# IDEA-CCNL/Fengshenbang-LM

Hardware: NVIDIA H100
Metric: tokens_per_sec (higher is better)
Workload: dtype bf16

## Files before the change

### fengshen-lm_b200/csrc/attention_bwd.cu

```cuda
#include "host_common.h"
#include "ptx.cuh"

namespace fsb {

int make_attn_tmap(CUtensorMap* tm, const void* base, int64_t row_stride, int64_t width, int64_t seq, int64_t batch,
                   int box_rows);

constexpr int AB_THREADS = 384;
constexpr int AB_BM = 128;
constexpr int AB_BN = 64;
constexpr int AB_NDIAG = AB_BM + AB_BN - 1;
constexpr int AB_DSTRIDE = 192;

struct AttBwdParams {
  const float* lse;
  const float* delta;
  const uint8_t* kv_mask;
  const float* rel_bias;
  float* dbias_part;
  __nv_bfloat16 *dq, *dk, *dv;
  int64_t dq_row_stride, dk_row_stride, dv_row_stride, dq_head_stride, dk_head_stride, dv_head_stride;
  int q_head_stride, k_head_stride, v_head_stride, do_head_stride;
  int seq_q, seq_kv, nheads, batch, causal;
  float scale, scale_log2;
};

template <int D>
__global__ void __launch_bounds__(256) attn_delta_kernel(const __nv_bfloat16* __restrict__ o,
                                                         const __nv_bfloat16* __restrict__ dout, float* __restrict__ delta,
                                                         int64_t o_row_stride, int64_t o_head_stride,
                                                         int64_t do_row_stride, int64_t do_head_stride, int batch, int seq,
                                                         int nheads) {
  constexpr int G = D / 8;
  const int64_t gid = (blockIdx.x * int64_t(blockDim.x) + threadIdx.x) / G;
  const int gl = threadIdx.x % G;
  const int64_t total = int64_t(batch) * seq * nheads;
  float s = 0.f;
  int64_t bs = 0; int h = 0;
  if (gid < total) {
    h = int(gid % nheads);
    bs = gid / nheads;
    float a[8], b[8];
    unpack8(*reinterpret_cast<const uint4*>(o + bs * o_row_stride + h * o_head_stride + gl * 8), a);
    unpack8(*reinterpret_cast<const uint4*>(dout + bs * do_row_stride + h * do_head_stride + gl * 8), b);
#pragma unroll
    for (int j = 0; j < 8; ++j) s += a[j] * b[j];
  }
#pragma unroll
  for (int off = G / 2; off > 0; off >>= 1) s += __shfl_xor_sync(0xffffffffu, s, off);
  if (gid < total && gl == 0) {
    const int64_t b = bs / seq, sq = bs % seq;
    delta[(b * nheads + h) * seq + sq] = s;
  }
}

template <int D, bool kDS>
struct AttBwdSmem {
  static constexpr int BIG_BYTES = AB_BM * D * 2;
  static constexpr int SML_BYTES = AB_BN * D * 2;
  static constexpr int STAGES = 3;
  static constexpr int OFF_BIG0 = 0;
  static constexpr int OFF_BIG1 = OFF_BIG0 + BIG_BYTES;
  static constexpr int OFF_SML0 = OFF_BIG1 + BIG_BYTES;
  static constexpr int OFF_SML1 = OFF_SML0 + STAGES * SML_BYTES;
  static constexpr int OFF_DS = OFF_SML1 + STAGES * SML_BYTES;
  static constexpr int OFF_BAR = OFF_DS + (kDS ? (AB_BM * (AB_BN + 1) * 4 + 15) / 16 * 16 : 0);
  static constexpr int NBAR = 1 + 2 * STAGES;
  static constexpr int TOTAL = OFF_BAR + NBAR * 8 + 1024;
  static_assert(TOTAL <= 232448, "exceeds the 227 KB of shared memory a block can opt into on sm_90");
};

template <int D>
__device__ __forceinline__ void wgmma_rs_acc(float (&o)[D / 2], const uint32_t (&a)[4], uint64_t db) {
  if constexpr (D == 128) wgmma_rs_n128<1>(o, a, db, 1u);
  else wgmma_rs_n64<1>(o, a, db, 1u);
}
__device__ __forceinline__ uint32_t kslice(int kk, int rows) { return (kk / 4) * (rows * 128) + (kk % 4) * 32; }
__device__ __forceinline__ void to_frag(const float (&x)[32], int kk, uint32_t (&a)[4]) {
#pragma unroll
  for (int r = 0; r < 4; ++r) {
    const int i = 2 * kk + (r >> 1), h = r & 1;
    a[r] = pack_bf16x2(x[4 * i + 2 * h], x[4 * i + 2 * h + 1]);
  }
}

template <int D, bool kBias>
__global__ void __launch_bounds__(AB_THREADS, 1)
attn_bwd_dq_kernel(const __grid_constant__ CUtensorMap tmQ, const __grid_constant__ CUtensorMap tmdO,
                   const __grid_constant__ CUtensorMap tmK, const __grid_constant__ CUtensorMap tmV,
                   const AttBwdParams p) {
  using S = AttBwdSmem<D, kBias>;
  constexpr int STAGES = S::STAGES;
  extern __shared__ uint8_t smem_raw[];
  uint8_t* smem = reinterpret_cast<uint8_t*>((reinterpret_cast<uintptr_t>(smem_raw) + 1023) & ~uintptr_t(1023));
  uint64_t* bars = reinterpret_cast<uint64_t*>(smem + S::OFF_BAR);
  uint64_t* big_full = bars;
  uint64_t* sml_full = big_full + 1;
  uint64_t* sml_empty = sml_full + STAGES;

  const int warp = threadIdx.x >> 5, lane = threadIdx.x & 31;
  const int tile = gridDim.x - 1 - blockIdx.x;
  const int head = blockIdx.y, b = blockIdx.z;
  const int q0 = tile * AB_BM;
  const int n_all = (p.seq_kv + AB_BN - 1) / AB_BN;
  const int n_steps = p.causal ? min(n_all, (min(q0 + AB_BM, p.seq_q) + AB_BN - 1) / AB_BN) : n_all;

  if (threadIdx.x == 0) {
    tma_prefetch_desc(&tmQ); tma_prefetch_desc(&tmdO); tma_prefetch_desc(&tmK); tma_prefetch_desc(&tmV);
    mbar_init(big_full, 1);
    for (int i = 0; i < STAGES; ++i) { mbar_init(&sml_full[i], 1); mbar_init(&sml_empty[i], 8); }
    fence_barrier_init();
  }
  __syncthreads();

  if (warp < 4) {
    reg_dec<24>();
    if (threadIdx.x == 0) {
      const int qc = head * p.q_head_stride, dc = head * p.do_head_stride;
      const int kc = head * p.k_head_stride, vc = head * p.v_head_stride;
      mbar_expect_tx(big_full, 2 * S::BIG_BYTES);
#pragma unroll
      for (int h = 0; h < D / 64; ++h) {
        tma_load_3d(smem + S::OFF_BIG0 + h * (AB_BM * 128), &tmQ, big_full, qc + h * 64, q0, b);
        tma_load_3d(smem + S::OFF_BIG1 + h * (AB_BM * 128), &tmdO, big_full, dc + h * 64, q0, b);
      }
      int st = 0; uint32_t ph = 0;
      for (int j = 0; j < n_steps; ++j) {
        mbar_wait(&sml_empty[st], ph ^ 1);
        mbar_expect_tx(&sml_full[st], 2 * S::SML_BYTES);
#pragma unroll
        for (int h = 0; h < D / 64; ++h) {
          tma_load_3d(smem + S::OFF_SML0 + st * S::SML_BYTES + h * (AB_BN * 128), &tmK, &sml_full[st], kc + h * 64, j * AB_BN, b);
          tma_load_3d(smem + S::OFF_SML1 + st * S::SML_BYTES + h * (AB_BN * 128), &tmV, &sml_full[st], vc + h * 64, j * AB_BN, b);
        }
        if (++st == STAGES) { st = 0; ph ^= 1; }
      }
    }
    return;
  }

  reg_inc<240>();
  const int wg = (threadIdx.x >> 7) - 1;
  const int r_lo = wg * 64 + (warp & 3) * 16 + (lane >> 2);
  const int cq = 2 * (lane & 3);
  const uint64_t dsc_q = make_smem_desc_sw128(smem_u32(smem + S::OFF_BIG0) + wg * (64 * 128), 0, 1024);
  const uint64_t dsc_do = make_smem_desc_sw128(smem_u32(smem + S::OFF_BIG1) + wg * (64 * 128), 0, 1024);
  const uint64_t dsc_k = make_smem_desc_sw128(smem_u32(smem + S::OFF_SML0), 0, 1024);
  const uint64_t dsc_v = make_smem_desc_sw128(smem_u32(smem + S::OFF_SML1), 0, 1024);
  const uint64_t dsc_kmn = make_smem_desc_sw128(smem_u32(smem + S::OFF_SML0), AB_BN * 128, 1024);
  const uint8_t* mrow = p.kv_mask ? p.kv_mask + int64_t(b) * p.seq_kv : nullptr;
  const int n_rel = p.seq_q + p.seq_kv - 1;
  int q_row[2], kmax[2];
  float lse[2], delta[2];
  const float* brow[2];
#pragma unroll
  for (int h = 0; h < 2; ++h) {
    q_row[h] = q0 + r_lo + 8 * h;
    const bool ok = q_row[h] < p.seq_q;
    const int64_t si = (int64_t(b) * p.nheads + head) * p.seq_q + q_row[h];
    lse[h] = ok ? p.lse[si] : INFINITY;
    delta[h] = ok ? p.delta[si] : 0.f;
    kmax[h] = p.causal ? min(q_row[h], p.seq_kv - 1) : p.seq_kv - 1;
    brow[h] = kBias ? p.rel_bias + int64_t(head) * n_rel + (p.seq_q - 1 - min(q_row[h], p.seq_q - 1)) : nullptr;
  }
  float* dpart = kBias && p.dbias_part ? p.dbias_part + ((int64_t(b) * p.nheads + head) * gridDim.x + tile) * n_all * AB_DSTRIDE
                                       : nullptr;
  float dq[D / 2];
#pragma unroll
  for (int i = 0; i < D / 2; ++i) dq[i] = 0.f;

  mbar_wait(big_full, 0);
  for (int j = 0; j < n_steps; ++j) {
    const int st = j % STAGES;
    const uint32_t ph = (j / STAGES) & 1;
    const uint64_t sto = uint64_t(st) * (S::SML_BYTES >> 4);
    float s[32], dp[32];
    mbar_wait(&sml_full[st], ph);
    wgmma_fence();
#pragma unroll
    for (int kk = 0; kk < D / 16; ++kk)
      wgmma_ss_n64<0, 0>(s, dsc_q + (kslice(kk, AB_BM) >> 4), dsc_k + sto + (kslice(kk, AB_BN) >> 4), kk != 0 ? 1u : 0u);
#pragma unroll
    for (int kk = 0; kk < D / 16; ++kk)
      wgmma_ss_n64<0, 0>(dp, dsc_do + (kslice(kk, AB_BM) >> 4), dsc_v + sto + (kslice(kk, AB_BN) >> 4), kk != 0 ? 1u : 0u);
    wgmma_commit();
    wgmma_wait<0>();
    wgmma_fence_acc(s);
    wgmma_fence_acc(dp);
    const int c0 = j * AB_BN;
    const bool need_mask = (p.causal && c0 + AB_BN - 1 > q0 + wg * 64) || (c0 + AB_BN > p.seq_kv) || mrow;
#pragma unroll
    for (int i = 0; i < 8; ++i) {
#pragma unroll
      for (int e = 0; e < 4; ++e) {
        const int h = e >> 1, col = c0 + 8 * i + cq + (e & 1);
        float x = s[4 * i + e] * p.scale_log2 - lse[h];
        if constexpr (kBias) x = fmaf(__ldg(brow[h] + min(col, p.seq_kv - 1)), 1.4426950408889634f, x);
        float pe = ex2_approx(x);
        if (need_mask) {
          bool keep = col <= kmax[h];
          if (mrow != nullptr && keep) keep = mrow[col] != 0;
          pe = keep ? pe : 0.f;
        }
        s[4 * i + e] = pe * (dp[4 * i + e] - delta[h]);
      }
    }
    if constexpr (kBias) {
      if (dpart != nullptr) {
        float* tds = reinterpret_cast<float*>(smem + S::OFF_DS);
#pragma unroll
        for (int i = 0; i < 8; ++i)
#pragma unroll
          for (int e = 0; e < 4; ++e) tds[(r_lo + 8 * (e >> 1)) * (AB_BN + 1) + 8 * i + cq + (e & 1)] = s[4 * i + e];
        bar_sync(1, 256);
        const int t = threadIdx.x - 128;
        if (t < AB_NDIAG) {
          const int o = t - (AB_BM - 1);
          float acc = 0.f;
          for (int r = max(0, -o); r < min(AB_BM, AB_BN - o); ++r) acc += tds[r * (AB_BN + 2) + o];
          dpart[int64_t(j) * AB_DSTRIDE + t] = acc;
        }
        bar_sync(1, 256);
      }
    }
    uint32_t a[AB_BN / 16][4];
#pragma unroll
    for (int kk = 0; kk < AB_BN / 16; ++kk) to_frag(s, kk, a[kk]);
    wgmma_fence();
#pragma unroll
    for (int kk = 0; kk < AB_BN / 16; ++kk) wgmma_rs_acc<D>(dq, a[kk], dsc_kmn + sto + ((kk * 2048) >> 4));
    wgmma_commit();
    wgmma_wait<0>();
    wgmma_fence_acc(dq);
    __syncwarp();
    if (lane == 0) mbar_arrive(&sml_empty[st]);
  }
#pragma unroll
  for (int h = 0; h < 2; ++h) {
    if (q_row[h] >= p.seq_q) continue;
    __nv_bfloat16* dqp = p.dq + (int64_t(b) * p.seq_q + q_row[h]) * p.dq_row_stride + int64_t(head) * p.dq_head_stride + cq;
#pragma unroll
    for (int i = 0; i < D / 8; ++i)
      *reinterpret_cast<uint32_t*>(dqp + 8 * i) = pack_bf16x2(dq[4 * i + 2 * h] * p.scale, dq[4 * i + 2 * h + 1] * p.scale);
  }
}

template <int D, bool kBias>
__global__ void __launch_bounds__(AB_THREADS, 1)
attn_bwd_dkv_kernel(const __grid_constant__ CUtensorMap tmK, const __grid_constant__ CUtensorMap tmV,
                    const __grid_constant__ CUtensorMap tmQ, const __grid_constant__ CUtensorMap tmdO,
                    const AttBwdParams p) {
  using S = AttBwdSmem<D, false>;
  constexpr int STAGES = S::STAGES;
  extern __shared__ uint8_t smem_raw[];
  uint8_t* smem = reinterpret_cast<uint8_t*>((reinterpret_cast<uintptr_t>(smem_raw) + 1023) & ~uintptr_t(1023));
  uint64_t* bars = reinterpret_cast<uint64_t*>(smem + S::OFF_BAR);
  uint64_t* big_full = bars;
  uint64_t* sml_full = big_full + 1;
  uint64_t* sml_empty = sml_full + STAGES;

  const int warp = threadIdx.x >> 5, lane = threadIdx.x & 31;
  const int tile = blockIdx.x;
  const int head = blockIdx.y, b = blockIdx.z;
  const int kv0 = tile * AB_BM;
  const int n_q = (p.seq_q + AB_BN - 1) / AB_BN;
  const int i_start = p.causal ? min(n_q, kv0 / AB_BN) : 0;
  const int n_steps = n_q - i_start;

  if (threadIdx.x == 0) {
    tma_prefetch_desc(&tmQ); tma_prefetch_desc(&tmdO); tma_prefetch_desc(&tmK); tma_prefetch_desc(&tmV);
    mbar_init(big_full, 1);
    for (int i = 0; i < STAGES; ++i) { mbar_init(&sml_full[i], 1); mbar_init(&sml_empty[i], 8); }
    fence_barrier_init();
  }
  __syncthreads();

  if (warp < 4) {
    reg_dec<24>();
    if (threadIdx.x == 0) {
      const int qc = head * p.q_head_stride, dc = head * p.do_head_stride;
      const int kc = head * p.k_head_stride, vc = head * p.v_head_stride;
      mbar_expect_tx(big_full, 2 * S::BIG_BYTES);
#pragma unroll
      for (int h = 0; h < D / 64; ++h) {
        tma_load_3d(smem + S::OFF_BIG0 + h * (AB_BM * 128), &tmK, big_full, kc + h * 64, kv0, b);
        tma_load_3d(smem + S::OFF_BIG1 + h * (AB_BM * 128), &tmV, big_full, vc + h * 64, kv0, b);
      }
      int st = 0; uint32_t ph = 0;
      for (int i = 0; i < n_steps; ++i) {
        mbar_wait(&sml_empty[st], ph ^ 1);
        mbar_expect_tx(&sml_full[st], 2 * S::SML_BYTES);
#pragma unroll
        for (int h = 0; h < D / 64; ++h) {
          tma_load_3d(smem + S::OFF_SML0 + st * S::SML_BYTES + h * (AB_BN * 128), &tmQ, &sml_full[st], qc + h * 64,
                      (i_start + i) * AB_BN, b);
          tma_load_3d(smem + S::OFF_SML1 + st * S::SML_BYTES + h * (AB_BN * 128), &tmdO, &sml_full[st], dc + h * 64,
                      (i_start + i) * AB_BN, b);
        }
        if (++st == STAGES) { st = 0; ph ^= 1; }
      }
    }
    return;
  }

  reg_inc<240>();
  const int wg = (threadIdx.x >> 7) - 1;
  const int r_lo = wg * 64 + (warp & 3) * 16 + (lane >> 2);
  const int cq = 2 * (lane & 3);
  const uint64_t dsc_k = make_smem_desc_sw128(smem_u32(smem + S::OFF_BIG0) + wg * (64 * 128), 0, 1024);
  const uint64_t dsc_v = make_smem_desc_sw128(smem_u32(smem + S::OFF_BIG1) + wg * (64 * 128), 0, 1024);
  const uint64_t dsc_q = make_smem_desc_sw128(smem_u32(smem + S::OFF_SML0), 0, 1024);
  const uint64_t dsc_do = make_smem_desc_sw128(smem_u32(smem + S::OFF_SML1), 0, 1024);
  const uint64_t dsc_qmn = make_smem_desc_sw128(smem_u32(smem + S::OFF_SML0), AB_BN * 128, 1024);
  const uint64_t dsc_domn = make_smem_desc_sw128(smem_u32(smem + S::OFF_SML1), AB_BN * 128, 1024);
  const int64_t stat_base = (int64_t(b) * p.nheads + head) * p.seq_q;
  const int n_rel = p.seq_q + p.seq_kv - 1;
  int kv_row[2];
  bool row_ok[2];
  const float* bkey[2];
#pragma unroll
  for (int h = 0; h < 2; ++h) {
    kv_row[h] = kv0 + r_lo + 8 * h;
    row_ok[h] = kv_row[h] < p.seq_kv && (p.kv_mask == nullptr || p.kv_mask[int64_t(b) * p.seq_kv + kv_row[h]] != 0);
    bkey[h] = kBias ? p.rel_bias + int64_t(head) * n_rel + (min(kv_row[h], p.seq_kv - 1) + p.seq_q - 1) : nullptr;
  }
  float dv[D / 2], dk[D / 2];
#pragma unroll
  for (int i = 0; i < D / 2; ++i) { dv[i] = 0.f; dk[i] = 0.f; }

  mbar_wait(big_full, 0);
  for (int i = 0; i < n_steps; ++i) {
    const int st = i % STAGES;
    const uint32_t ph = (i / STAGES) & 1;
    const uint64_t sto = uint64_t(st) * (S::SML_BYTES >> 4);
    const int qt0 = (i_start + i) * AB_BN;
    float s[32], dp[32];
    mbar_wait(&sml_full[st], ph);
    wgmma_fence();
#pragma unroll
    for (int kk = 0; kk < D / 16; ++kk)
      wgmma_ss_n64<0, 0>(s, dsc_k + (kslice(kk, AB_BM) >> 4), dsc_q + sto + (kslice(kk, AB_BN) >> 4), kk != 0 ? 1u : 0u);
#pragma unroll
    for (int kk = 0; kk < D / 16; ++kk)
      wgmma_ss_n64<0, 0>(dp, dsc_v + (kslice(kk, AB_BM) >> 4), dsc_do + sto + (kslice(kk, AB_BN) >> 4), kk != 0 ? 1u : 0u);
    wgmma_commit();
    wgmma_wait<0>();
    wgmma_fence_acc(s);
    wgmma_fence_acc(dp);
    const bool need_causal = p.causal && (qt0 < kv0 + AB_BM - 1);
#pragma unroll
    for (int ii = 0; ii < 8; ++ii) {
#pragma unroll
      for (int c = 0; c < 2; ++c) {
        const int qi = qt0 + 8 * ii + cq + c;
        const bool q_ok = qi < p.seq_q;
        const float lse_c = q_ok ? __ldg(p.lse + stat_base + qi) : INFINITY;
        const float del_c = q_ok ? __ldg(p.delta + stat_base + qi) : 0.f;
#pragma unroll
        for (int h = 0; h < 2; ++h) {
          const int e = 2 * h + c;
          float arg = s[4 * ii + e] * p.scale_log2 - lse_c;
          if constexpr (kBias) arg = fmaf(__ldg(bkey[h] - min(qi, p.seq_q - 1)), 1.4426950408889634f, arg);
          float x = ex2_approx(arg);
          const bool keep = row_ok[h] && !(need_causal && qi < kv_row[h]);
          x = keep ? x : 0.f;
          s[4 * ii + e] = x;
          dp[4 * ii + e] = x * (dp[4 * ii + e] - del_c);
        }
      }
    }
    uint32_t pa[AB_BN / 16][4], da[AB_BN / 16][4];
#pragma unroll
    for (int kk = 0; kk < AB_BN / 16; ++kk) { to_frag(s, kk, pa[kk]); to_frag(dp, kk, da[kk]); }
    wgmma_fence();
#pragma unroll
    for (int kk = 0; kk < AB_BN / 16; ++kk) wgmma_rs_acc<D>(dv, pa[kk], dsc_domn + sto + ((kk * 2048) >> 4));
#pragma unroll
    for (int kk = 0; kk < AB_BN / 16; ++kk) wgmma_rs_acc<D>(dk, da[kk], dsc_qmn + sto + ((kk * 2048) >> 4));
    wgmma_commit();
    wgmma_wait<0>();
    wgmma_fence_acc(dv);
    wgmma_fence_acc(dk);
    __syncwarp();
    if (lane == 0) mbar_arrive(&sml_empty[st]);
  }
#pragma unroll
  for (int h = 0; h < 2; ++h) {
    if (kv_row[h] >= p.seq_kv) continue;
    __nv_bfloat16* dvp = p.dv + (int64_t(b) * p.seq_kv + kv_row[h]) * p.dv_row_stride + int64_t(head) * p.dv_head_stride + cq;
    __nv_bfloat16* dkp = p.dk + (int64_t(b) * p.seq_kv + kv_row[h]) * p.dk_row_stride + int64_t(head) * p.dk_head_stride + cq;
#pragma unroll
    for (int i = 0; i < D / 8; ++i) {
      *reinterpret_cast<uint32_t*>(dvp + 8 * i) = pack_bf16x2(dv[4 * i + 2 * h], dv[4 * i + 2 * h + 1]);
      *reinterpret_cast<uint32_t*>(dkp + 8 * i) = pack_bf16x2(dk[4 * i + 2 * h] * p.scale, dk[4 * i + 2 * h + 1] * p.scale);
    }
  }
}

__global__ void __launch_bounds__(128) attn_dbias_reduce_kernel(const float* __restrict__ part, float* __restrict__ part2,
                                                                int batch, int nheads, int seq_q, int seq_kv, int causal,
                                                                int n_qtiles, int bsplit) {
  const int n_rel = seq_q + seq_kv - 1;
  const int i = blockIdx.x * blockDim.x + threadIdx.x;
  const int h = blockIdx.y, sp = blockIdx.z;
  if (i >= n_rel) return;
  const int d = i - (seq_q - 1);
  const int n_all = (seq_kv + AB_BN - 1) / AB_BN;
  const int b0 = int(int64_t(batch) * sp / bsplit), b1 = int(int64_t(batch) * (sp + 1) / bsplit);
  float acc = 0.f;
  for (int b = b0; b < b1; ++b) {
    for (int tile = 0; tile < n_qtiles; ++tile) {
      const int q0 = tile * AB_BM;
      const int n_steps = causal ? min(n_all, (min(q0 + AB_BM, seq_q) + AB_BN - 1) / AB_BN) : n_all;
      const float* base = part + ((int64_t(b) * nheads + h) * n_qtiles + tile) * n_all * AB_DSTRIDE;
      const int hi = d + q0 + (AB_BM - 1), lo = d + q0 - (AB_BN - 1);
      if (hi < 0) continue;
      const int j_lo = lo <= 0 ? 0 : (lo + AB_BN - 1) / AB_BN, j_hi = min(n_steps - 1, hi / AB_BN);
      for (int j = j_lo; j <= j_hi; ++j) acc += base[int64_t(j) * AB_DSTRIDE + (hi - j * AB_BN)];
    }
  }
  part2[(int64_t(sp) * nheads + h) * n_rel + i] = acc;
}
__global__ void __launch_bounds__(128) attn_dbias_final_kernel(const float* __restrict__ part2, float* __restrict__ dbias,
                                                               int nheads, int n_rel, int bsplit) {
  const int i = blockIdx.x * blockDim.x + threadIdx.x;
  const int h = blockIdx.y;
  if (i >= n_rel) return;
  float acc = dbias[int64_t(h) * n_rel + i];
  for (int sp = 0; sp < bsplit; ++sp) acc += part2[(int64_t(sp) * nheads + h) * n_rel + i];
  dbias[int64_t(h) * n_rel + i] = acc;
}
static inline int dbias_bsplit(int batch) { return batch < 16 ? batch : 16; }
static inline size_t dbias_part_floats(int64_t batch, int64_t seq_q, int64_t seq_kv, int nheads) {
  const int64_t n_qt = (seq_q + AB_BM - 1) / AB_BM, n_all = (seq_kv + AB_BN - 1) / AB_BN;
  return size_t(batch) * nheads * n_qt * n_all * AB_DSTRIDE;
}

template <int D, bool kBias>
static int launch_attn_bwd(const void* q, const void* k, const void* v, const void* o, const void* dout,
                           int64_t q_rs, int64_t k_rs, int64_t v_rs, int64_t o_rs, int64_t do_rs, int64_t o_hs,
                           float* delta, AttBwdParams& p, float* drel_bias, float* part2, cudaStream_t st) {
  using SQ = AttBwdSmem<D, kBias>;
  using SK = AttBwdSmem<D, false>;
  static bool configured = false;
  if (!configured) {
    cudaError_t e1 = cudaFuncSetAttribute(attn_bwd_dq_kernel<D, kBias>, cudaFuncAttributeMaxDynamicSharedMemorySize, SQ::TOTAL);
    cudaError_t e2 = cudaFuncSetAttribute(attn_bwd_dkv_kernel<D, kBias>, cudaFuncAttributeMaxDynamicSharedMemorySize, SK::TOTAL);
    if (e1 != cudaSuccess || e2 != cudaSuccess) {
      set_error("sdpa_bwd: cudaFuncSetAttribute(%d / %d) failed", SQ::TOTAL, SK::TOTAL);
      return FSB_ERR_CUDA;
    }
    configured = true;
  }
  {
    const int64_t groups = int64_t(p.batch) * p.seq_q * p.nheads;
    const int64_t threads = groups * (D / 8);
    attn_delta_kernel<D><<<unsigned((threads + 255) / 256), 256, 0, st>>>(
        (const __nv_bfloat16*)o, (const __nv_bfloat16*)dout, delta, o_rs, o_hs, do_rs, p.do_head_stride, p.batch, p.seq_q,
        p.nheads);
    FSB_CUDA_LAUNCH_CHECK();
  }
  CUtensorMap tq128, tdo128, tk64, tv64, tk128, tv128, tq64, tdo64;
  int rc;
  const int64_t wq = int64_t(p.nheads - 1) * p.q_head_stride + D, wk = int64_t(p.nheads - 1) * p.k_head_stride + D;
  const int64_t wv = int64_t(p.nheads - 1) * p.v_head_stride + D, wdo = int64_t(p.nheads - 1) * p.do_head_stride + D;
  if ((rc = make_attn_tmap(&tq128, q, q_rs, wq, p.seq_q, p.batch, AB_BM))) return rc;
  if ((rc = make_attn_tmap(&tdo128, dout, do_rs, wdo, p.seq_q, p.batch, AB_BM))) return rc;
  if ((rc = make_attn_tmap(&tk64, k, k_rs, wk, p.seq_kv, p.batch, AB_BN))) return rc;
  if ((rc = make_attn_tmap(&tv64, v, v_rs, wv, p.seq_kv, p.batch, AB_BN))) return rc;
  if ((rc = make_attn_tmap(&tk128, k, k_rs, wk, p.seq_kv, p.batch, AB_BM))) return rc;
  if ((rc = make_attn_tmap(&tv128, v, v_rs, wv, p.seq_kv, p.batch, AB_BM))) return rc;
  if ((rc = make_attn_tmap(&tq64, q, q_rs, wq, p.seq_q, p.batch, AB_BN))) return rc;
  if ((rc = make_attn_tmap(&tdo64, dout, do_rs, wdo, p.seq_q, p.batch, AB_BN))) return rc;
  {
    dim3 grid((p.seq_q + AB_BM - 1) / AB_BM, p.nheads, p.batch);
    attn_bwd_dq_kernel<D, kBias><<<grid, AB_THREADS, SQ::TOTAL, st>>>(tq128, tdo128, tk64, tv64, p);
    FSB_CUDA_LAUNCH_CHECK();
    if (kBias && drel_bias != nullptr) {
      const int n_rel = p.seq_q + p.seq_kv - 1, bs = dbias_bsplit(p.batch);
      attn_dbias_reduce_kernel<<<dim3((n_rel + 127) / 128, p.nheads, bs), 128, 0, st>>>(
          p.dbias_part, part2, p.batch, p.nheads, p.seq_q, p.seq_kv, p.causal, int(grid.x), bs);
      FSB_CUDA_LAUNCH_CHECK();
      attn_dbias_final_kernel<<<dim3((n_rel + 127) / 128, p.nheads), 128, 0, st>>>(part2, drel_bias, p.nheads, n_rel, bs);
      FSB_CUDA_LAUNCH_CHECK();
    }
  }
  {
    dim3 grid((p.seq_kv + AB_BM - 1) / AB_BM, p.nheads, p.batch);
    attn_bwd_dkv_kernel<D, kBias><<<grid, AB_THREADS, SK::TOTAL, st>>>(tk128, tv128, tq64, tdo64, p);
    FSB_CUDA_LAUNCH_CHECK();
  }
  return FSB_OK;
}

}

using namespace fsb;

extern "C" int fsb_sdpa_bwd(const void* q, const void* k, const void* v, const void* o, const void* dout,
                            const float* lse, float* delta, void* dq, void* dk, void* dv, int64_t batch, int64_t seq_q,
                            int64_t seq_kv, int nheads, int head_dim, int64_t q_row_stride, int64_t k_row_stride,
                            int64_t v_row_stride, int64_t o_row_stride, int64_t do_row_stride, int64_t dq_row_stride,
                            int64_t dk_row_stride, int64_t dv_row_stride, int64_t q_head_stride, int64_t k_head_stride,
                            int64_t v_head_stride, int64_t o_head_stride, int64_t do_head_stride,
                            int64_t dq_head_stride, int64_t dk_head_stride, int64_t dv_head_stride, float scale,
                            int causal, const uint8_t* kv_mask, const float* rel_bias, float* drel_bias, void* workspace,
                            size_t workspace_bytes, fsb_stream_t st) {
  FSB_REQUIRE(q && k && v && o && dout && lse && delta && dq && dk && dv, "sdpa_bwd: null pointer");
  FSB_REQUIRE(head_dim == 64 || head_dim == 128, "sdpa_bwd: head_dim %d unsupported (64 or 128)", head_dim);
  FSB_REQUIRE(batch > 0 && seq_q > 0 && seq_kv > 0 && nheads > 0 && batch < 65536 && nheads < 65536, "sdpa_bwd: bad dims");
  FSB_REQUIRE(!causal || seq_q == seq_kv, "sdpa_bwd: causal needs seq_q == seq_kv");
  FSB_REQUIRE(aligned16(q) && aligned16(k) && aligned16(v) && aligned16(o) && aligned16(dout) && aligned16(dq) &&
                  aligned16(dk) && aligned16(dv),
              "sdpa_bwd: 16-byte alignment required");
  FSB_REQUIRE((q_row_stride | k_row_stride | v_row_stride | o_row_stride | do_row_stride | dq_row_stride |
               dk_row_stride | dv_row_stride | q_head_stride | k_head_stride | v_head_stride | o_head_stride |
               do_head_stride | dq_head_stride | dk_head_stride | dv_head_stride) % 8 == 0,
              "sdpa_bwd: strides must be multiples of 8 elements");
  FSB_REQUIRE(drel_bias == nullptr || rel_bias != nullptr, "sdpa_bwd: drel_bias without rel_bias");
  AttBwdParams p;
  p.lse = lse; p.delta = delta; p.kv_mask = kv_mask;
  p.rel_bias = rel_bias; p.dbias_part = nullptr;
  float* part2 = nullptr;
  if (drel_bias != nullptr) {
    const size_t need = fsb_sdpa_bwd_workspace_bytes(batch, seq_q, seq_kv, nheads);
    FSB_REQUIRE(workspace != nullptr && workspace_bytes >= need && aligned16(workspace),
                "sdpa_bwd: the bias gradient needs a %zu-byte workspace (fsb_sdpa_bwd_workspace_bytes); got %zu", need,
                workspace_bytes);
    p.dbias_part = static_cast<float*>(workspace);
    part2 = p.dbias_part + dbias_part_floats(batch, seq_q, seq_kv, nheads);
  }
  p.dq = (__nv_bfloat16*)dq; p.dk = (__nv_bfloat16*)dk; p.dv = (__nv_bfloat16*)dv;
  p.dq_row_stride = dq_row_stride; p.dk_row_stride = dk_row_stride; p.dv_row_stride = dv_row_stride;
  p.dq_head_stride = dq_head_stride; p.dk_head_stride = dk_head_stride; p.dv_head_stride = dv_head_stride;
  p.q_head_stride = int(q_head_stride); p.k_head_stride = int(k_head_stride); p.v_head_stride = int(v_head_stride);
  p.do_head_stride = int(do_head_stride);
  p.seq_q = int(seq_q); p.seq_kv = int(seq_kv); p.nheads = nheads; p.batch = int(batch); p.causal = causal;
  p.scale = scale; p.scale_log2 = scale * 1.4426950408889634f;
#define FSB_BWD(DD, BB)                                                                                                  \
  launch_attn_bwd<DD, BB>(q, k, v, o, dout, q_row_stride, k_row_stride, v_row_stride, o_row_stride, do_row_stride,       \
                          o_head_stride, delta, p, drel_bias, part2, (cudaStream_t)st)
  if (rel_bias != nullptr) return head_dim == 128 ? FSB_BWD(128, true) : FSB_BWD(64, true);
  return head_dim == 128 ? FSB_BWD(128, false) : FSB_BWD(64, false);
#undef FSB_BWD
}

extern "C" size_t fsb_sdpa_bwd_workspace_bytes(int64_t batch, int64_t seq_q, int64_t seq_kv, int nheads) {
  if (batch <= 0 || seq_q <= 0 || seq_kv <= 0 || nheads <= 0) return 0;
  return (fsb::dbias_part_floats(batch, seq_q, seq_kv, nheads) +
          size_t(fsb::dbias_bsplit(int(batch))) * nheads * size_t(seq_q + seq_kv - 1)) * sizeof(float);
}
```

### fengshen-lm_b200/csrc/ptx.cuh

```cuda
#pragma once
#include <cuda.h>
#include <cuda_bf16.h>
#include <cuda_runtime.h>
#include <stdint.h>

namespace fsb {

__device__ __forceinline__ uint32_t smem_u32(const void* p) {
  return static_cast<uint32_t>(__cvta_generic_to_shared(p));
}

__device__ __forceinline__ void mbar_init(uint64_t* bar, uint32_t count) {
  asm volatile("mbarrier.init.shared::cta.b64 [%0], %1;" ::"r"(smem_u32(bar)), "r"(count) : "memory");
}
__device__ __forceinline__ void fence_barrier_init() {
  asm volatile("fence.mbarrier_init.release.cluster;" ::: "memory");
}
__device__ __forceinline__ void fence_proxy_async() {
  asm volatile("fence.proxy.async.shared::cta;" ::: "memory");
}
__device__ __forceinline__ void mbar_expect_tx(uint64_t* bar, uint32_t bytes) {
  asm volatile("mbarrier.arrive.expect_tx.shared::cta.b64 _, [%0], %1;" ::"r"(smem_u32(bar)), "r"(bytes)
               : "memory");
}
__device__ __forceinline__ void mbar_arrive(uint64_t* bar) {
  asm volatile("mbarrier.arrive.shared::cta.b64 _, [%0];" ::"r"(smem_u32(bar)) : "memory");
}
__device__ __forceinline__ bool mbar_try_wait(uint64_t* bar, uint32_t parity) {
  uint32_t ok;
  asm volatile(
      "{\n\t"
      ".reg .pred p;\n\t"
      "mbarrier.try_wait.parity.shared::cta.b64 p, [%1], %2;\n\t"
      "selp.b32 %0, 1, 0, p;\n\t"
      "}"
      : "=r"(ok)
      : "r"(smem_u32(bar)), "r"(parity)
      : "memory");
  return ok != 0;
}
__device__ __forceinline__ bool mbar_test(uint64_t* bar, uint32_t parity) {
  uint32_t ok;
  asm volatile(
      "{\n\t"
      ".reg .pred p;\n\t"
      "mbarrier.test_wait.parity.shared::cta.b64 p, [%1], %2;\n\t"
      "selp.b32 %0, 1, 0, p;\n\t"
      "}"
      : "=r"(ok)
      : "r"(smem_u32(bar)), "r"(parity)
      : "memory");
  return ok != 0;
}
__device__ __forceinline__ void mbar_wait(uint64_t* bar, uint32_t parity) {
  while (!mbar_try_wait(bar, parity)) {
  }
}

__device__ __forceinline__ void tma_prefetch_desc(const CUtensorMap* m) {
  asm volatile("prefetch.tensormap [%0];" ::"l"(reinterpret_cast<uint64_t>(m)) : "memory");
}
__device__ __forceinline__ void tma_load_2d(void* smem_dst, const CUtensorMap* m, uint64_t* bar, int c0, int c1) {
  asm volatile(
      "cp.async.bulk.tensor.2d.shared::cluster.global.mbarrier::complete_tx::bytes [%0], [%1, {%3, %4}], [%2];"
      ::"r"(smem_u32(smem_dst)), "l"(reinterpret_cast<uint64_t>(m)), "r"(smem_u32(bar)), "r"(c0), "r"(c1)
      : "memory");
}
__device__ __forceinline__ void tma_load_3d(void* smem_dst, const CUtensorMap* m, uint64_t* bar, int c0, int c1,
                                            int c2) {
  asm volatile(
      "cp.async.bulk.tensor.3d.shared::cluster.global.mbarrier::complete_tx::bytes [%0], [%1, {%3, %4, %5}], [%2];"
      ::"r"(smem_u32(smem_dst)), "l"(reinterpret_cast<uint64_t>(m)), "r"(smem_u32(bar)), "r"(c0), "r"(c1), "r"(c2)
      : "memory");
}
constexpr uint64_t kL2EvictNormal = 0x1000000000000000ull, kL2EvictFirst = 0x12F0000000000000ull,
                   kL2EvictLast = 0x14F0000000000000ull;
__device__ __forceinline__ void tma_load_3d_hint(void* smem_dst, const CUtensorMap* m, uint64_t* bar, int c0, int c1, int c2,
                                                 uint64_t policy) {
  asm volatile(
      "cp.async.bulk.tensor.3d.shared::cluster.global.mbarrier::complete_tx::bytes.L2::cache_hint [%0], [%1, {%3, %4, %5}], [%2], %6;"
      ::"r"(smem_u32(smem_dst)), "l"(reinterpret_cast<uint64_t>(m)), "r"(smem_u32(bar)), "r"(c0), "r"(c1), "r"(c2), "l"(policy)
      : "memory");
}
__device__ __forceinline__ void tma_store_3d_hint(const CUtensorMap* m, const void* smem_src, int c0, int c1, int c2,
                                                  uint64_t policy) {
  asm volatile("cp.async.bulk.tensor.3d.global.shared::cta.bulk_group.L2::cache_hint [%0, {%2, %3, %4}], [%1], %5;" ::"l"(
                   reinterpret_cast<uint64_t>(m)),
               "r"(smem_u32(smem_src)), "r"(c0), "r"(c1), "r"(c2), "l"(policy)
               : "memory");
}
__device__ __forceinline__ void tma_store_2d(const CUtensorMap* m, const void* smem_src, int c0, int c1) {
  asm volatile("cp.async.bulk.tensor.2d.global.shared::cta.bulk_group [%0, {%2, %3}], [%1];" ::"l"(
                   reinterpret_cast<uint64_t>(m)),
               "r"(smem_u32(smem_src)), "r"(c0), "r"(c1)
               : "memory");
}
__device__ __forceinline__ void tma_store_3d(const CUtensorMap* m, const void* smem_src, int c0, int c1, int c2) {
  asm volatile("cp.async.bulk.tensor.3d.global.shared::cta.bulk_group [%0, {%2, %3, %4}], [%1];" ::"l"(
                   reinterpret_cast<uint64_t>(m)),
               "r"(smem_u32(smem_src)), "r"(c0), "r"(c1), "r"(c2)
               : "memory");
}
__device__ __forceinline__ void tma_store_commit() { asm volatile("cp.async.bulk.commit_group;" ::: "memory"); }
template <int N>
__device__ __forceinline__ void tma_store_wait_read() {
  asm volatile("cp.async.bulk.wait_group.read %0;" ::"n"(N) : "memory");
}
template <int N>
__device__ __forceinline__ void tma_store_wait() {
  asm volatile("cp.async.bulk.wait_group %0;" ::"n"(N) : "memory");
}

__device__ __forceinline__ void wgmma_fence() { asm volatile("wgmma.fence.sync.aligned;" ::: "memory"); }
__device__ __forceinline__ void wgmma_commit() { asm volatile("wgmma.commit_group.sync.aligned;" ::: "memory"); }
template <int N>
__device__ __forceinline__ void wgmma_wait() { asm volatile("wgmma.wait_group.sync.aligned %0;" ::"n"(N) : "memory"); }
template <int R>
__device__ __forceinline__ void wgmma_fence_acc(float (&d)[R]) {
#pragma unroll
  for (int i = 0; i < R; ++i) asm volatile("" : "+f"(d[i])::"memory");
}
template <int N> __device__ __forceinline__ void reg_inc() { asm volatile("setmaxnreg.inc.sync.aligned.u32 %0;" ::"n"(N)); }
template <int N> __device__ __forceinline__ void reg_dec() { asm volatile("setmaxnreg.dec.sync.aligned.u32 %0;" ::"n"(N)); }
__device__ __forceinline__ void bar_sync(int id, int n) { asm volatile("bar.sync %0, %1;" ::"r"(id), "r"(n) : "memory"); }
__device__ __forceinline__ float ex2_approx(float x) {
  float y;
  asm("ex2.approx.ftz.f32 %0, %1;" : "=f"(y) : "f"(x));
  return y;
}

__device__ __forceinline__ uint64_t make_smem_desc_sw128(uint32_t saddr, uint32_t lbo, uint32_t sbo) {
  uint64_t d = 0;
  d |= static_cast<uint64_t>((saddr & 0x3FFFF) >> 4);
  d |= static_cast<uint64_t>((lbo >> 4) & 0x3FFF) << 16;
  d |= static_cast<uint64_t>((sbo >> 4) & 0x3FFF) << 32;
  d |= static_cast<uint64_t>(1) << 62;
  return d;
}

template <int kTA, int kTB>
__device__ __forceinline__ void wgmma_ss_n64(float (&d)[32], uint64_t da, uint64_t db, uint32_t accumulate) {
  asm volatile(
      "{\n.reg .pred p;\nsetp.ne.b32 p, %34, 0;\n"
      "wgmma.mma_async.sync.aligned.m64n64k16.f32.bf16.bf16 {%0, %1, %2, %3, %4, %5, %6, %7, %8, %9, %10, %11, %12, %13, %14, %15, %16, %17, %18, %19, %20, %21, %22, %23, %24, %25, %26, %27, %28, %29, %30, %31}, %32, %33, p, 1, 1, %35, %36;\n}"
      : "+f"(d[0]), "+f"(d[1]), "+f"(d[2]), "+f"(d[3]), "+f"(d[4]), "+f"(d[5]), "+f"(d[6]), "+f"(d[7]), "+f"(d[8]), "+f"(d[9]), "+f"(d[10]), "+f"(d[11]), "+f"(d[12]), "+f"(d[13]), "+f"(d[14]), "+f"(d[15]), "+f"(d[16]), "+f"(d[17]), "+f"(d[18]), "+f"(d[19]), "+f"(d[20]), "+f"(d[21]), "+f"(d[22]), "+f"(d[23]), "+f"(d[24]), "+f"(d[25]), "+f"(d[26]), "+f"(d[27]), "+f"(d[28]), "+f"(d[29]), "+f"(d[30]), "+f"(d[31])
      : "l"(da), "l"(db), "r"(accumulate), "n"(kTA), "n"(kTB));
}
template <int kTB>
__device__ __forceinline__ void wgmma_rs_n64(float (&d)[32], const uint32_t (&a)[4], uint64_t db, uint32_t accumulate) {
  asm volatile(
      "{\n.reg .pred p;\nsetp.ne.b32 p, %37, 0;\n"
      "wgmma.mma_async.sync.aligned.m64n64k16.f32.bf16.bf16 {%0, %1, %2, %3, %4, %5, %6, %7, %8, %9, %10, %11, %12, %13, %14, %15, %16, %17, %18, %19, %20, %21, %22, %23, %24, %25, %26, %27, %28, %29, %30, %31}, {%32, %33, %34, %35}, %36, p, 1, 1, %38;\n}"
      : "+f"(d[0]), "+f"(d[1]), "+f"(d[2]), "+f"(d[3]), "+f"(d[4]), "+f"(d[5]), "+f"(d[6]), "+f"(d[7]), "+f"(d[8]), "+f"(d[9]), "+f"(d[10]), "+f"(d[11]), "+f"(d[12]), "+f"(d[13]), "+f"(d[14]), "+f"(d[15]), "+f"(d[16]), "+f"(d[17]), "+f"(d[18]), "+f"(d[19]), "+f"(d[20]), "+f"(d[21]), "+f"(d[22]), "+f"(d[23]), "+f"(d[24]), "+f"(d[25]), "+f"(d[26]), "+f"(d[27]), "+f"(d[28]), "+f"(d[29]), "+f"(d[30]), "+f"(d[31])
      : "r"(a[0]), "r"(a[1]), "r"(a[2]), "r"(a[3]), "l"(db), "r"(accumulate), "n"(kTB));
}
template <int kTA, int kTB>
__device__ __forceinline__ void wgmma_ss_n128(float (&d)[64], uint64_t da, uint64_t db, uint32_t accumulate) {
  asm volatile(
      "{\n.reg .pred p;\nsetp.ne.b32 p, %66, 0;\n"
      "wgmma.mma_async.sync.aligned.m64n128k16.f32.bf16.bf16 {%0, %1, %2, %3, %4, %5, %6, %7, %8, %9, %10, %11, %12, %13, %14, %15, %16, %17, %18, %19, %20, %21, %22, %23, %24, %25, %26, %27, %28, %29, %30, %31, %32, %33, %34, %35, %36, %37, %38, %39, %40, %41, %42, %43, %44, %45, %46, %47, %48, %49, %50, %51, %52, %53, %54, %55, %56, %57, %58, %59, %60, %61, %62, %63}, %64, %65, p, 1, 1, %67, %68;\n}"
      : "+f"(d[0]), "+f"(d[1]), "+f"(d[2]), "+f"(d[3]), "+f"(d[4]), "+f"(d[5]), "+f"(d[6]), "+f"(d[7]), "+f"(d[8]), "+f"(d[9]), "+f"(d[10]), "+f"(d[11]), "+f"(d[12]), "+f"(d[13]), "+f"(d[14]), "+f"(d[15]), "+f"(d[16]), "+f"(d[17]), "+f"(d[18]), "+f"(d[19]), "+f"(d[20]), "+f"(d[21]), "+f"(d[22]), "+f"(d[23]), "+f"(d[24]), "+f"(d[25]), "+f"(d[26]), "+f"(d[27]), "+f"(d[28]), "+f"(d[29]), "+f"(d[30]), "+f"(d[31]), "+f"(d[32]), "+f"(d[33]), "+f"(d[34]), "+f"(d[35]), "+f"(d[36]), "+f"(d[37]), "+f"(d[38]), "+f"(d[39]), "+f"(d[40]), "+f"(d[41]), "+f"(d[42]), "+f"(d[43]), "+f"(d[44]), "+f"(d[45]), "+f"(d[46]), "+f"(d[47]), "+f"(d[48]), "+f"(d[49]), "+f"(d[50]), "+f"(d[51]), "+f"(d[52]), "+f"(d[53]), "+f"(d[54]), "+f"(d[55]), "+f"(d[56]), "+f"(d[57]), "+f"(d[58]), "+f"(d[59]), "+f"(d[60]), "+f"(d[61]), "+f"(d[62]), "+f"(d[63])
      : "l"(da), "l"(db), "r"(accumulate), "n"(kTA), "n"(kTB));
}
template <int kTB>
__device__ __forceinline__ void wgmma_rs_n128(float (&d)[64], const uint32_t (&a)[4], uint64_t db, uint32_t accumulate) {
  asm volatile(
      "{\n.reg .pred p;\nsetp.ne.b32 p, %69, 0;\n"
      "wgmma.mma_async.sync.aligned.m64n128k16.f32.bf16.bf16 {%0, %1, %2, %3, %4, %5, %6, %7, %8, %9, %10, %11, %12, %13, %14, %15, %16, %17, %18, %19, %20, %21, %22, %23, %24, %25, %26, %27, %28, %29, %30, %31, %32, %33, %34, %35, %36, %37, %38, %39, %40, %41, %42, %43, %44, %45, %46, %47, %48, %49, %50, %51, %52, %53, %54, %55, %56, %57, %58, %59, %60, %61, %62, %63}, {%64, %65, %66, %67}, %68, p, 1, 1, %70;\n}"
      : "+f"(d[0]), "+f"(d[1]), "+f"(d[2]), "+f"(d[3]), "+f"(d[4]), "+f"(d[5]), "+f"(d[6]), "+f"(d[7]), "+f"(d[8]), "+f"(d[9]), "+f"(d[10]), "+f"(d[11]), "+f"(d[12]), "+f"(d[13]), "+f"(d[14]), "+f"(d[15]), "+f"(d[16]), "+f"(d[17]), "+f"(d[18]), "+f"(d[19]), "+f"(d[20]), "+f"(d[21]), "+f"(d[22]), "+f"(d[23]), "+f"(d[24]), "+f"(d[25]), "+f"(d[26]), "+f"(d[27]), "+f"(d[28]), "+f"(d[29]), "+f"(d[30]), "+f"(d[31]), "+f"(d[32]), "+f"(d[33]), "+f"(d[34]), "+f"(d[35]), "+f"(d[36]), "+f"(d[37]), "+f"(d[38]), "+f"(d[39]), "+f"(d[40]), "+f"(d[41]), "+f"(d[42]), "+f"(d[43]), "+f"(d[44]), "+f"(d[45]), "+f"(d[46]), "+f"(d[47]), "+f"(d[48]), "+f"(d[49]), "+f"(d[50]), "+f"(d[51]), "+f"(d[52]), "+f"(d[53]), "+f"(d[54]), "+f"(d[55]), "+f"(d[56]), "+f"(d[57]), "+f"(d[58]), "+f"(d[59]), "+f"(d[60]), "+f"(d[61]), "+f"(d[62]), "+f"(d[63])
      : "r"(a[0]), "r"(a[1]), "r"(a[2]), "r"(a[3]), "l"(db), "r"(accumulate), "n"(kTB));
}
template <int kTA, int kTB>
__device__ __forceinline__ void wgmma_ss_n256(float (&d)[128], uint64_t da, uint64_t db, uint32_t accumulate) {
  asm volatile(
      "{\n.reg .pred p;\nsetp.ne.b32 p, %130, 0;\n"
      "wgmma.mma_async.sync.aligned.m64n256k16.f32.bf16.bf16 {%0, %1, %2, %3, %4, %5, %6, %7, %8, %9, %10, %11, %12, %13, %14, %15, %16, %17, %18, %19, %20, %21, %22, %23, %24, %25, %26, %27, %28, %29, %30, %31, %32, %33, %34, %35, %36, %37, %38, %39, %40, %41, %42, %43, %44, %45, %46, %47, %48, %49, %50, %51, %52, %53, %54, %55, %56, %57, %58, %59, %60, %61, %62, %63, %64, %65, %66, %67, %68, %69, %70, %71, %72, %73, %74, %75, %76, %77, %78, %79, %80, %81, %82, %83, %84, %85, %86, %87, %88, %89, %90, %91, %92, %93, %94, %95, %96, %97, %98, %99, %100, %101, %102, %103, %104, %105, %106, %107, %108, %109, %110, %111, %112, %113, %114, %115, %116, %117, %118, %119, %120, %121, %122, %123, %124, %125, %126, %127}, %128, %129, p, 1, 1, %131, %132;\n}"
      : "+f"(d[0]), "+f"(d[1]), "+f"(d[2]), "+f"(d[3]), "+f"(d[4]), "+f"(d[5]), "+f"(d[6]), "+f"(d[7]), "+f"(d[8]), "+f"(d[9]), "+f"(d[10]), "+f"(d[11]), "+f"(d[12]), "+f"(d[13]), "+f"(d[14]), "+f"(d[15]), "+f"(d[16]), "+f"(d[17]), "+f"(d[18]), "+f"(d[19]), "+f"(d[20]), "+f"(d[21]), "+f"(d[22]), "+f"(d[23]), "+f"(d[24]), "+f"(d[25]), "+f"(d[26]), "+f"(d[27]), "+f"(d[28]), "+f"(d[29]), "+f"(d[30]), "+f"(d[31]), "+f"(d[32]), "+f"(d[33]), "+f"(d[34]), "+f"(d[35]), "+f"(d[36]), "+f"(d[37]), "+f"(d[38]), "+f"(d[39]), "+f"(d[40]), "+f"(d[41]), "+f"(d[42]), "+f"(d[43]), "+f"(d[44]), "+f"(d[45]), "+f"(d[46]), "+f"(d[47]), "+f"(d[48]), "+f"(d[49]), "+f"(d[50]), "+f"(d[51]), "+f"(d[52]), "+f"(d[53]), "+f"(d[54]), "+f"(d[55]), "+f"(d[56]), "+f"(d[57]), "+f"(d[58]), "+f"(d[59]), "+f"(d[60]), "+f"(d[61]), "+f"(d[62]), "+f"(d[63]), "+f"(d[64]), "+f"(d[65]), "+f"(d[66]), "+f"(d[67]), "+f"(d[68]), "+f"(d[69]), "+f"(d[70]), "+f"(d[71]), "+f"(d[72]), "+f"(d[73]), "+f"(d[74]), "+f"(d[75]), "+f"(d[76]), "+f"(d[77]), "+f"(d[78]), "+f"(d[79]), "+f"(d[80]), "+f"(d[81]), "+f"(d[82]), "+f"(d[83]), "+f"(d[84]), "+f"(d[85]), "+f"(d[86]), "+f"(d[87]), "+f"(d[88]), "+f"(d[89]), "+f"(d[90]), "+f"(d[91]), "+f"(d[92]), "+f"(d[93]), "+f"(d[94]), "+f"(d[95]), "+f"(d[96]), "+f"(d[97]), "+f"(d[98]), "+f"(d[99]), "+f"(d[100]), "+f"(d[101]), "+f"(d[102]), "+f"(d[103]), "+f"(d[104]), "+f"(d[105]), "+f"(d[106]), "+f"(d[107]), "+f"(d[108]), "+f"(d[109]), "+f"(d[110]), "+f"(d[111]), "+f"(d[112]), "+f"(d[113]), "+f"(d[114]), "+f"(d[115]), "+f"(d[116]), "+f"(d[117]), "+f"(d[118]), "+f"(d[119]), "+f"(d[120]), "+f"(d[121]), "+f"(d[122]), "+f"(d[123]), "+f"(d[124]), "+f"(d[125]), "+f"(d[126]), "+f"(d[127])
      : "l"(da), "l"(db), "r"(accumulate), "n"(kTA), "n"(kTB));
}
template <int kTB>
__device__ __forceinline__ void wgmma_rs_n256(float (&d)[128], const uint32_t (&a)[4], uint64_t db, uint32_t accumulate) {
  asm volatile(
      "{\n.reg .pred p;\nsetp.ne.b32 p, %133, 0;\n"
      "wgmma.mma_async.sync.aligned.m64n256k16.f32.bf16.bf16 {%0, %1, %2, %3, %4, %5, %6, %7, %8, %9, %10, %11, %12, %13, %14, %15, %16, %17, %18, %19, %20, %21, %22, %23, %24, %25, %26, %27, %28, %29, %30, %31, %32, %33, %34, %35, %36, %37, %38, %39, %40, %41, %42, %43, %44, %45, %46, %47, %48, %49, %50, %51, %52, %53, %54, %55, %56, %57, %58, %59, %60, %61, %62, %63, %64, %65, %66, %67, %68, %69, %70, %71, %72, %73, %74, %75, %76, %77, %78, %79, %80, %81, %82, %83, %84, %85, %86, %87, %88, %89, %90, %91, %92, %93, %94, %95, %96, %97, %98, %99, %100, %101, %102, %103, %104, %105, %106, %107, %108, %109, %110, %111, %112, %113, %114, %115, %116, %117, %118, %119, %120, %121, %122, %123, %124, %125, %126, %127}, {%128, %129, %130, %131}, %132, p, 1, 1, %134;\n}"
      : "+f"(d[0]), "+f"(d[1]), "+f"(d[2]), "+f"(d[3]), "+f"(d[4]), "+f"(d[5]), "+f"(d[6]), "+f"(d[7]), "+f"(d[8]), "+f"(d[9]), "+f"(d[10]), "+f"(d[11]), "+f"(d[12]), "+f"(d[13]), "+f"(d[14]), "+f"(d[15]), "+f"(d[16]), "+f"(d[17]), "+f"(d[18]), "+f"(d[19]), "+f"(d[20]), "+f"(d[21]), "+f"(d[22]), "+f"(d[23]), "+f"(d[24]), "+f"(d[25]), "+f"(d[26]), "+f"(d[27]), "+f"(d[28]), "+f"(d[29]), "+f"(d[30]), "+f"(d[31]), "+f"(d[32]), "+f"(d[33]), "+f"(d[34]), "+f"(d[35]), "+f"(d[36]), "+f"(d[37]), "+f"(d[38]), "+f"(d[39]), "+f"(d[40]), "+f"(d[41]), "+f"(d[42]), "+f"(d[43]), "+f"(d[44]), "+f"(d[45]), "+f"(d[46]), "+f"(d[47]), "+f"(d[48]), "+f"(d[49]), "+f"(d[50]), "+f"(d[51]), "+f"(d[52]), "+f"(d[53]), "+f"(d[54]), "+f"(d[55]), "+f"(d[56]), "+f"(d[57]), "+f"(d[58]), "+f"(d[59]), "+f"(d[60]), "+f"(d[61]), "+f"(d[62]), "+f"(d[63]), "+f"(d[64]), "+f"(d[65]), "+f"(d[66]), "+f"(d[67]), "+f"(d[68]), "+f"(d[69]), "+f"(d[70]), "+f"(d[71]), "+f"(d[72]), "+f"(d[73]), "+f"(d[74]), "+f"(d[75]), "+f"(d[76]), "+f"(d[77]), "+f"(d[78]), "+f"(d[79]), "+f"(d[80]), "+f"(d[81]), "+f"(d[82]), "+f"(d[83]), "+f"(d[84]), "+f"(d[85]), "+f"(d[86]), "+f"(d[87]), "+f"(d[88]), "+f"(d[89]), "+f"(d[90]), "+f"(d[91]), "+f"(d[92]), "+f"(d[93]), "+f"(d[94]), "+f"(d[95]), "+f"(d[96]), "+f"(d[97]), "+f"(d[98]), "+f"(d[99]), "+f"(d[100]), "+f"(d[101]), "+f"(d[102]), "+f"(d[103]), "+f"(d[104]), "+f"(d[105]), "+f"(d[106]), "+f"(d[107]), "+f"(d[108]), "+f"(d[109]), "+f"(d[110]), "+f"(d[111]), "+f"(d[112]), "+f"(d[113]), "+f"(d[114]), "+f"(d[115]), "+f"(d[116]), "+f"(d[117]), "+f"(d[118]), "+f"(d[119]), "+f"(d[120]), "+f"(d[121]), "+f"(d[122]), "+f"(d[123]), "+f"(d[124]), "+f"(d[125]), "+f"(d[126]), "+f"(d[127])
      : "r"(a[0]), "r"(a[1]), "r"(a[2]), "r"(a[3]), "l"(db), "r"(accumulate), "n"(kTB));
}

__device__ __forceinline__ uint32_t pack_bf16x2(float lo, float hi) {
  __nv_bfloat162 v = __floats2bfloat162_rn(lo, hi);
  return *reinterpret_cast<uint32_t*>(&v);
}
__device__ __forceinline__ float bf16lo(uint32_t u) { return __uint_as_float(u << 16); }
__device__ __forceinline__ float bf16hi(uint32_t u) { return __uint_as_float(u & 0xFFFF0000u); }

__device__ __forceinline__ void unpack8(const uint4& q, float (&f)[8]) {
  f[0] = bf16lo(q.x); f[1] = bf16hi(q.x); f[2] = bf16lo(q.y); f[3] = bf16hi(q.y);
  f[4] = bf16lo(q.z); f[5] = bf16hi(q.z); f[6] = bf16lo(q.w); f[7] = bf16hi(q.w);
}
__device__ __forceinline__ uint4 pack8(const float (&f)[8]) {
  uint4 q;
  q.x = pack_bf16x2(f[0], f[1]); q.y = pack_bf16x2(f[2], f[3]);
  q.z = pack_bf16x2(f[4], f[5]); q.w = pack_bf16x2(f[6], f[7]);
  return q;
}
__device__ __forceinline__ float round_bf16(float x) { return __bfloat162float(__float2bfloat16(x)); }

}
```

Baseline: 448,300.

## Stage LSE/delta in smem via producer warp, skip masked causal tiles, register-resident K/V

```diff
diff --git a/fengshen-lm_b200/csrc/attention_bwd.cu b/fengshen-lm_b200/csrc/attention_bwd.cu
--- a/fengshen-lm_b200/csrc/attention_bwd.cu
+++ b/fengshen-lm_b200/csrc/attention_bwd.cu
@@ -64,7 +64,8 @@
   static constexpr int OFF_SML0 = OFF_BIG1 + BIG_BYTES;
   static constexpr int OFF_SML1 = OFF_SML0 + STAGES * SML_BYTES;
   static constexpr int OFF_DS = OFF_SML1 + STAGES * SML_BYTES;
-  static constexpr int OFF_BAR = OFF_DS + (kDS ? (AB_BM * (AB_BN + 1) * 4 + 15) / 16 * 16 : 0);
+  static constexpr int OFF_STAT = OFF_DS + (kDS ? (AB_BM * (AB_BN + 1) * 4 + 15) / 16 * 16 : 0);
+  static constexpr int OFF_BAR = OFF_STAT + STAGES * 2 * AB_BN * 4;
   static constexpr int NBAR = 1 + 2 * STAGES;
   static constexpr int TOTAL = OFF_BAR + NBAR * 8 + 1024;
   static_assert(TOTAL <= 232448, "exceeds the 227 KB of shared memory a block can opt into on sm_90");
@@ -176,6 +177,11 @@
     const uint64_t sto = uint64_t(st) * (S::SML_BYTES >> 4);
     float s[32], dp[32];
     mbar_wait(&sml_full[st], ph);
+    if (!kBias && p.causal && j * AB_BN > q0 + wg * 64 + 63) {
+      __syncwarp();
+      if (lane == 0) mbar_arrive(&sml_empty[st]);
+      continue;
+    }
     wgmma_fence();
 #pragma unroll
     for (int kk = 0; kk < D / 16; ++kk)
@@ -266,11 +272,12 @@
   const int n_q = (p.seq_q + AB_BN - 1) / AB_BN;
   const int i_start = p.causal ? min(n_q, kv0 / AB_BN) : 0;
   const int n_steps = n_q - i_start;
+  const int64_t stat_base = (int64_t(b) * p.nheads + head) * p.seq_q;
 
   if (threadIdx.x == 0) {
     tma_prefetch_desc(&tmQ); tma_prefetch_desc(&tmdO); tma_prefetch_desc(&tmK); tma_prefetch_desc(&tmV);
     mbar_init(big_full, 1);
-    for (int i = 0; i < STAGES; ++i) { mbar_init(&sml_full[i], 1); mbar_init(&sml_empty[i], 8); }
+    for (int i = 0; i < STAGES; ++i) { mbar_init(&sml_full[i], 2); mbar_init(&sml_empty[i], 8); }
     fence_barrier_init();
   }
   __syncthreads();
@@ -297,6 +304,21 @@
           tma_load_3d(smem + S::OFF_SML1 + st * S::SML_BYTES + h * (AB_BN * 128), &tmdO, &sml_full[st], dc + h * 64,
                       (i_start + i) * AB_BN, b);
         }
+        if (++st == STAGES) { st = 0; ph ^= 1; }
+      }
+    } else if (warp == 1) {
+      int st = 0; uint32_t ph = 0;
+      for (int i = 0; i < n_steps; ++i) {
+        mbar_wait(&sml_empty[st], ph ^ 1);
+        float* stat = reinterpret_cast<float*>(smem + S::OFF_STAT) + st * 2 * AB_BN;
+        for (int c = lane; c < AB_BN; c += 32) {
+          const int qi = (i_start + i) * AB_BN + c;
+          const bool q_ok = qi < p.seq_q;
+          stat[c] = q_ok ? __ldg(p.lse + stat_base + qi) : INFINITY;
+          stat[AB_BN + c] = q_ok ? __ldg(p.delta + stat_base + qi) : 0.f;
+        }
+        __syncwarp();
+        if (lane == 0) mbar_arrive(&sml_full[st]);
         if (++st == STAGES) { st = 0; ph ^= 1; }
       }
     }
@@ -313,7 +335,6 @@
   const uint64_t dsc_do = make_smem_desc_sw128(smem_u32(smem + S::OFF_SML1), 0, 1024);
   const uint64_t dsc_qmn = make_smem_desc_sw128(smem_u32(smem + S::OFF_SML0), AB_BN * 128, 1024);
   const uint64_t dsc_domn = make_smem_desc_sw128(smem_u32(smem + S::OFF_SML1), AB_BN * 128, 1024);
-  const int64_t stat_base = (int64_t(b) * p.nheads + head) * p.seq_q;
   const int n_rel = p.seq_q + p.seq_kv - 1;
   int kv_row[2];
   bool row_ok[2];
@@ -329,20 +350,41 @@
   for (int i = 0; i < D / 2; ++i) { dv[i] = 0.f; dk[i] = 0.f; }
 
   mbar_wait(big_full, 0);
+  constexpr bool kRegA = D == 64;
+  uint32_t ka[kRegA ? D / 16 : 1][4], va[kRegA ? D / 16 : 1][4];
+  if constexpr (kRegA) {
+#pragma unroll
+    for (int kk = 0; kk < D / 16; ++kk) {
+      load_frag_sw128(smem + S::OFF_BIG0, AB_BM, r_lo, kk, cq, ka[kk]);
+      load_frag_sw128(smem + S::OFF_BIG1, AB_BM, r_lo, kk, cq, va[kk]);
+    }
+  }
   for (int i = 0; i < n_steps; ++i) {
     const int st = i % STAGES;
     const uint32_t ph = (i / STAGES) & 1;
     const uint64_t sto = uint64_t(st) * (S::SML_BYTES >> 4);
     const int qt0 = (i_start + i) * AB_BN;
+    const float* stat = reinterpret_cast<const float*>(smem + S::OFF_STAT) + st * 2 * AB_BN;
     float s[32], dp[32];
     mbar_wait(&sml_full[st], ph);
+    if (!kBias && p.causal && qt0 + AB_BN - 1 < kv0 + wg * 64) {
+      __syncwarp();
+      if (lane == 0) mbar_arrive(&sml_empty[st]);
+      continue;
+    }
     wgmma_fence();
 #pragma unroll
-    for (int kk = 0; kk < D / 16; ++kk)
-      wgmma_ss_n64<0, 0>(s, dsc_k + (kslice(kk, AB_BM) >> 4), dsc_q + sto + (kslice(kk, AB_BN) >> 4), kk != 0 ? 1u : 0u);
-#pragma unroll
-    for (int kk = 0; kk < D / 16; ++kk)
-      wgmma_ss_n64<0, 0>(dp, dsc_v + (kslice(kk, AB_BM) >> 4), dsc_do + sto + (kslice(kk, AB_BN) >> 4), kk != 0 ? 1u : 0u);
+    for (int kk = 0; kk < D / 16; ++kk) {
+      const uint64_t bq = dsc_q + sto + (kslice(kk, AB_BN) >> 4);
+      if constexpr (kRegA) wgmma_rs_n64<0>(s, ka[kk], bq, kk != 0 ? 1u : 0u);
+      else wgmma_ss_n64<0, 0>(s, dsc_k + (kslice(kk, AB_BM) >> 4), bq, kk != 0 ? 1u : 0u);
+    }
+#pragma unroll
+    for (int kk = 0; kk < D / 16; ++kk) {
+      const uint64_t bdo = dsc_do + sto + (kslice(kk, AB_BN) >> 4);
+      if constexpr (kRegA) wgmma_rs_n64<0>(dp, va[kk], bdo, kk != 0 ? 1u : 0u);
+      else wgmma_ss_n64<0, 0>(dp, dsc_v + (kslice(kk, AB_BM) >> 4), bdo, kk != 0 ? 1u : 0u);
+    }
     wgmma_commit();
     wgmma_wait<0>();
     wgmma_fence_acc(s);
@@ -353,9 +395,7 @@
 #pragma unroll
       for (int c = 0; c < 2; ++c) {
         const int qi = qt0 + 8 * ii + cq + c;
-        const bool q_ok = qi < p.seq_q;
-        const float lse_c = q_ok ? __ldg(p.lse + stat_base + qi) : INFINITY;
-        const float del_c = q_ok ? __ldg(p.delta + stat_base + qi) : 0.f;
+        const float lse_c = stat[8 * ii + cq + c], del_c = stat[AB_BN + 8 * ii + cq + c];
 #pragma unroll
         for (int h = 0; h < 2; ++h) {
           const int e = 2 * h + c;
diff --git a/fengshen-lm_b200/csrc/ptx.cuh b/fengshen-lm_b200/csrc/ptx.cuh
--- a/fengshen-lm_b200/csrc/ptx.cuh
+++ b/fengshen-lm_b200/csrc/ptx.cuh
@@ -187,6 +187,15 @@
       : "r"(a[0]), "r"(a[1]), "r"(a[2]), "r"(a[3]), "l"(db), "r"(accumulate), "n"(kTB));
 }
 
+__device__ __forceinline__ void load_frag_sw128(const uint8_t* tile, int rows, int row, int kk, int cq, uint32_t (&a)[4]) {
+#pragma unroll
+  for (int r = 0; r < 4; ++r) {
+    const int rr = row + 8 * (r & 1), col = 16 * (kk % 4) + cq + 8 * (r >> 1);
+    a[r] = *reinterpret_cast<const uint32_t*>(tile + (kk / 4) * (rows * 128) + rr * 128 + (((col >> 3) ^ (rr & 7)) << 4) +
+                                              (col & 7) * 2);
+  }
+}
+
 __device__ __forceinline__ uint32_t pack_bf16x2(float lo, float hi) {
   __nv_bfloat162 v = __floats2bfloat162_rn(lo, hi);
   return *reinterpret_cast<uint32_t*>(&v);
```

Result: no change. 448,900, median of 6 (+0.1%).
